# jgkellymit/GENIE-SMEM

Measured on AMD Instinct MI355X. Metric: query-bases/sec SMEM discovery, 100kb ref x 150bp reads; bit-exact SMEM set, higher is better.
Workload: dtype u8/int32 (2-bit packed bases, int32 SA rows; f64 only in the RMI predict)

## Files before the change

genie-smem_amd/csrc/kernels.hip:

```cpp
#include <hip/hip_runtime.h>

#include <algorithm>
#include <cstdio>
#include <cstdlib>
#include <mutex>
#include <string>
#include <unordered_map>

#include "genie_internal.h"

namespace genie {

namespace {

constexpr int kWave = 64;

__device__ __forceinline__ int rfl(int v) { return __builtin_amdgcn_readfirstlane(v); }
__device__ __forceinline__ void set_wave_priority(int i)
{
    switch (i & 3) {
    case 0: __builtin_amdgcn_s_setprio(0); break;
    case 1: __builtin_amdgcn_s_setprio(1); break;
    case 2: __builtin_amdgcn_s_setprio(2); break;
    default: __builtin_amdgcn_s_setprio(3); break;
    }
}

__device__ __forceinline__ void scalar_touch_lines(const void *p, uint32_t bytes)
{
    uint32_t d, off;
    asm volatile("s_mov_b32 %[off], 0\n"
                 "1:\n\t"
                 "s_load_dword %[d], %[p], %[off]\n\t"
                 "s_add_u32 %[off], %[off], 64\n\t"
                 "s_cmp_lt_u32 %[off], %[n]\n\t"
                 "s_cbranch_scc1 1b\n\t"
                 "s_waitcnt lgkmcnt(0)"
                 : [d] "=&s"(d), [off] "=&s"(off)
                 : [p] "s"(reinterpret_cast<uint64_t>(p) & ~3ull), [n] "s"(bytes)
                 : "scc", "memory");
}

__device__ __forceinline__ void wave_lds_fence()
{
    __builtin_amdgcn_fence(__ATOMIC_ACQ_REL, "wavefront");
    __builtin_amdgcn_wave_barrier();
}

__device__ __forceinline__ uint64_t funnel(uint64_t w0, uint64_t w1, int sh )
{
// ... 1 lines not shown
}

__device__ __forceinline__ uint64_t qwin(const uint64_t *qp, int pos)
{
    int i = pos >> 5;
    return funnel(qp[i], qp[i + 1], (pos & 31) * 2);
}

__device__ __forceinline__ uint64_t rwin(const RefRec *ref, int pos)
{
    const ulonglong2 v = *reinterpret_cast<const ulonglong2 *>(ref + (pos >> 5));
    return funnel(v.x, v.y, (pos & 31) * 2);
}

struct QWords {
    const uint64_t *p;
    __device__ __forceinline__ uint64_t win(int pos) const { return qwin(p, pos); }
};
struct QRecs {
    const RefRec *p;
    __device__ __forceinline__ uint64_t win(int pos) const { return rwin(p, pos); }
};
struct QPlain {
    const uint64_t *p;
    __device__ __forceinline__ uint64_t win(int pos) const
    {
        typedef uint64_t u64x2 __attribute__((ext_vector_type(2)));
        typedef u64x2 u64x2_a8 __attribute__((aligned(8)));
        const u64x2 v = *reinterpret_cast<const u64x2_a8 *>(p + (pos >> 5));
        return funnel(v.x, v.y, (pos & 31) * 2);
    }
};

template <class D>
__device__ __forceinline__ uint32_t dir_lb(const DevIndex &ix, const D dir, uint32_t code, int m)
{
    const uint32_t x = code << (2 * (ix.P - m));
    uint32_t v = dir[x];
#pragma unroll
    for (int l = 0; l < GENIE_MAX_DIR_BITS; l++)
        if (l >= m && l < ix.P && ix.padtail[l] == x) v--;
    return v;
}

template <class D>
__device__ __forceinline__ uint32_t dir_ub(const DevIndex &ix, const D dir, uint32_t code, int m)
{
    const uint32_t x = (code + 1) << (2 * (ix.P - m));
    uint32_t v = dir[x];
#pragma unroll
    for (int l = 1; l < GENIE_MAX_DIR_BITS; l++)
        if (l < ix.P && ix.padtail[l] == x) v--;
    return v;
}

struct Cmp {
    int l;
    bool less;
};

template <class Q>
__device__ __forceinline__ Cmp cmp_suffix(const DevIndex &ix, const Q qp, int a, int m, int s, int skip)
{
    const int avail = ix.n - s;
    const int lim = m < avail ? m : avail;
    int l = skip;
    bool less = false;
    bool diff = false;
    while (l < lim) {
        const uint64_t xq = qp.win(a + l), xr = rwin(ix.ref, s + l);
        const uint64_t x = xq ^ xr;
        if (x) {
            l += __clzll((long long)x) >> 1;
            less = xr < xq;
            diff = true;
            break;
        }
        l += 32;
    }
    if (!diff || l >= lim) {
        l = lim;
        less = lim < m;
    }
    return {l, less};
}

template <class Q>
__device__ __forceinline__ Cmp cmp_rec(const DevIndex &ix, const Q qp, int a, int m, const SaRec rec, uint64_t xq)
{
    const int avail = ix.n - rec.s;
    const int lim = m < avail ? m : avail;
    int l = ix.P;
    bool less;
    const uint64_t x = xq ^ rec.key;
    if (x) {
        l += __clzll((long long)x) >> 1;
        less = rec.key < xq;
        if (l >= lim) { l = lim; less = lim < m; }
    } else if (l + 32 >= lim) {
        l = lim;
        less = lim < m;
    } else {
        return cmp_suffix(ix, qp, a, m, rec.s, l + 32);
    }
    return {l, less};
}

__device__ __forceinline__ int pick_probe(int lo, int hi, uint32_t xq32, uint32_t vlo, uint32_t vhi, int step)
{
    const int n = hi - lo;
    if ((step & 1) || n <= 2 || vhi <= vlo) return (lo + hi) >> 1;
    if (xq32 <= vlo) return lo;
    if (xq32 >= vhi) return hi - 1;
    const float f = (float)(xq32 - vlo) / (float)(vhi - vlo);
    int mid = lo + (int)(f * (float)n);
    mid = mid < lo ? lo : (mid > hi - 1 ? hi - 1 : mid);
    return mid;
}

typedef uint32_t nt_u4 __attribute__((ext_vector_type(4)));
typedef nt_u4 nt_u4_unaligned __attribute__((aligned(1)));
__device__ __forceinline__ void store_nt(void *dst, uint4 v)
{
    __builtin_nontemporal_store(nt_u4{v.x, v.y, v.z, v.w}, reinterpret_cast<nt_u4 *>(dst));
}

__device__ __forceinline__ SaRec load_rec(const SaRec *sa, int row)
{
    int4 v = *reinterpret_cast<const int4 *>(sa + row);
    asm volatile("" : "+v"(v.x), "+v"(v.y), "+v"(v.z), "+v"(v.w));
    SaRec r;
    r.s = v.x;
    r.pad = 0;
    r.key = ((uint64_t)(uint32_t)v.w << 32) | (uint32_t)v.z;
    return r;
}

__device__ __forceinline__ bool lut_probe(const DevIndex &ix, uint32_t code, int &lo, int &hi)
{
    uint32_t p = (uint32_t)(((uint64_t)(code * 0x9E3779B1u) * (uint64_t)ix.lut_slots) >> 32);
    for (uint32_t tries = 0; tries < ix.lut_slots; tries++) {
        const int4 v = *reinterpret_cast<const int4 *>(ix.lut + p);
        if (v.y < 0) return false;
        if ((uint32_t)v.x == code) { lo = v.y; hi = v.z; return true; }
        p = p + 1 == ix.lut_slots ? 0 : p + 1;
    }
    return false;
}

__device__ __forceinline__ double rmi_predict(const DevIndex &ix, const RmiModel *leaf, int leaf_cnt, uint32_t code,
                                              int *leaf_idx = nullptr)
{
    const double x = (double)code;
    double p = 0.0;
    int idx = 0;
    for (int l = 0; l < ix.nlev; l++) {
        if (leaf_idx && l == ix.nlev - 1) *leaf_idx = idx;
        double2 m;
        if (leaf && l == ix.nlev - 1 && idx < leaf_cnt) m = *reinterpret_cast<const double2 *>(leaf + idx);
        else m = *reinterpret_cast<const double2 *>(ix.rmi + ix.rmi_off[l] + idx);
        p = __dadd_rn(__dmul_rn(m.x, x), m.y);
        const int scale = ix.rmi_scale[l];
        idx = !(p > 0.0) ? 0 : (p >= (double)scale ? scale - 1 : (int)p);
    }
    return p;
}

__device__ __forceinline__ int kmer_cmp_row(const DevIndex &ix, int r, uint32_t code)
{
    const int s = ix.sa[r].s;
    const int avail = ix.n - s;
    if (avail == 0) return -1;
    const uint64_t w = rwin(ix.ref, s);
    if (avail >= ix.K) {
        const uint32_t rc = (uint32_t)(w >> (64 - 2 * ix.K));
        return rc < code ? -1 : (rc > code ? 1 : 0);
    }
    const uint32_t rc = (uint32_t)(w >> (64 - 2 * avail));
    const uint32_t qc = code >> (2 * (ix.K - avail));
    return rc <= qc ? -1 : 1;
}

__device__ __forceinline__ bool rmi_lookup(const DevIndex &ix, const RmiModel *leaf, uint32_t code, int &lo, int &hi,
                                           double *pred_out)
{
    int leaf_idx = 0;
    const double p = rmi_predict(ix, leaf, 0, code, &leaf_idx);
    if (pred_out) *pred_out = p;
    const int rows = ix.n + 1;
    const int r0 = !(p > 0.0) ? 0 : (p >= (double)rows ? rows - 1 : (int)p);
    int L, R;
    bool fenced = false;
    if (ix.rmi_err) {
        const int e = ix.rmi_err[leaf_idx];
        L = r0 - e < 0 ? 0 : r0 - e;
        R = r0 + e + 1 > rows ? rows : r0 + e + 1;
        int l2 = L, r2 = R;
        while (l2 < r2) {
            const int mid = (l2 + r2) >> 1;
            if (kmer_cmp_row(ix, mid, code) < 0) l2 = mid + 1; else r2 = mid;
        }
        if (l2 < rows && kmer_cmp_row(ix, l2, code) == 0 && (l2 > L || L == 0 || kmer_cmp_row(ix, l2 - 1, code) < 0)) {
            L = R = l2;
            fenced = true;
        }
    }
    if (!fenced) {
    if (kmer_cmp_row(ix, r0, code) < 0) {
        L = r0 + 1;
        R = rows;
        for (int step = 1;; step <<= 1) {
            const int pr = r0 + step;
            if (pr >= rows) break;
            if (kmer_cmp_row(ix, pr, code) < 0) L = pr + 1;
            else { R = pr; break; }
        }
    } else {
        R = r0;
        L = 0;
        for (int step = 1;; step <<= 1) {
            const int pr = r0 - step;
            if (pr < 0) break;
            if (kmer_cmp_row(ix, pr, code) < 0) { L = pr + 1; break; }
            R = pr;
        }
    }
    }
    while (L < R) {
        const int mid = (L + R) >> 1;
        if (kmer_cmp_row(ix, mid, code) < 0) L = mid + 1; else R = mid;
    }
    const int first = L;
    if (first >= rows || kmer_cmp_row(ix, first, code) != 0) { lo = first; hi = first - 1; return false; }
    int a = first, b = rows;
    for (int step = 1;; step <<= 1) {
        const int pr = first + step;
        if (pr >= rows) break;
        if (kmer_cmp_row(ix, pr, code) == 0) a = pr;
        else { b = pr; break; }
    }
    while (b - a > 1) {
        const int mid = (a + b) >> 1;
        if (kmer_cmp_row(ix, mid, code) == 0) a = mid; else b = mid;
    }
    lo = first;
    hi = a;
    return true;
}

template <class Q>
__device__ __forceinline__ int2 sa_interval(const DevIndex &ix, const uint32_t *dir, const Q qp, int a, int m)
{
    if (m == 0) return make_int2(0, ix.n);
    const int P = ix.P;
    const uint64_t w = qp.win(a);
    if (m <= P) {
        const uint32_t code = (uint32_t)(w >> (64 - 2 * m));
        const int lb = (int)dir_lb(ix, dir, code, m), ub = (int)dir_ub(ix, dir, code, m);
        return lb < ub ? make_int2(lb, ub - 1) : make_int2(-1, -1);
    }
    const uint64_t xq = qp.win(a + P);
    int lo, hi, h;
    int known = -1;
    if (ix.P2 && m >= ix.P2) {
        int4 hd = *reinterpret_cast<const int4 *>(ix.dir2 + (uint32_t)(w >> (64 - 2 * ix.P2)));
        asm volatile("" : "+v"(hd.x), "+v"(hd.y), "+v"(hd.z), "+v"(hd.w));
        const uint32_t cnt = (uint32_t)hd.y & ~kHeadShort;
        if (cnt == 0) return make_int2(-1, -1);
        lo = hd.x;
        hi = h = hd.x + (int)cnt;
        const uint64_t key = ((uint64_t)(uint32_t)hd.w << 32) | (uint32_t)hd.z;
        const uint64_t x = xq ^ key;
        if (!((uint32_t)hd.y & kHeadShort) && (x != 0 || m <= P + 32)) {
            const int l = x ? P + (__clzll((long long)x) >> 1) : m;
            if (l >= m) { h = lo; known = lo; }
            else if (key < xq) lo = lo + 1;
            else h = lo;
        }
    } else {
        const uint32_t b = (uint32_t)(w >> (64 - 2 * P));
        lo = (int)dir[b];
        hi = h = (int)dir_ub(ix, dir, b, P);
    }
    uint32_t vlo = 0, vhi = 0xFFFFFFFFu;
// ... 930 lines not shown
```

genie-smem_amd/csrc/match_table_body.inc:

```
    static_assert(!(PK && RC), "both strands of 2-bit packed reads are not built");
    typedef uint32_t __attribute__((aligned(1))) u32_unaligned;
    extern __shared__ __align__(16) uint8_t smem[];
    const int lane = threadIdx.x & (kWave - 1);
    const int wave = rfl((int)(threadIdx.x >> 6));
    const int waves_per_block = blockDim.x >> 6;
    const int dbg = (flags >> 8) & 63;
    const int sched = flags >> 16;
    const bool look_up_all = (flags & 1) != 0;
    const int FS = fwd_stride;
    const int K = ix.K;
    const int P2 = ix.P2;
    const int DW = mt_short_row_dwords(max_len, qp_recs);
    const int DWp = mt_pack_dwords(max_len);
    const int QL = mt_quads(max_len);
    const int nquads = grp * QL;
    const __amdgpu_buffer_rsrc_t mtab =
        __builtin_amdgcn_make_buffer_rsrc(const_cast<MatchRec *>(ix.mtab), 0, (int)mtab_bytes, 0x00020000);
    const __amdgpu_buffer_rsrc_t ov =
        __builtin_amdgcn_make_buffer_rsrc(const_cast<MatchOv16 *>(ix.ov), 0, ix.ov_entries * (int)sizeof(MatchOv16), 0x00020000);

    uint8_t *wb = smem + wave * mt_wave_bytes(grp, max_len, qp_recs, FS);
    uint32_t *Dp = reinterpret_cast<uint32_t *>(wb);
    int *Ls = reinterpret_cast<int *>(wb + mt_r16(grp * DW * 4));
    uint8_t *fwL = reinterpret_cast<uint8_t *>(Ls) + 64;
    uint16_t *sl = reinterpret_cast<uint16_t *>(fwL + mt_r16(grp * FS));
    uint16_t *qa = reinterpret_cast<uint16_t *>(reinterpret_cast<uint8_t *>(sl) + mt_r16(mt_slow_cap(grp, max_len) * 2));
    uint16_t *qb = qa + grp * mt_quads(max_len);
    for (int i = lane; i < grp * DW; i += kWave) Dp[i] = 0;
    const uint8_t *reads_end = reads + (RC ? N >> 1 : N) * (long long)stride;

    const int pu = (int)(((uint32_t)lane * (uint32_t)(65536 / DWp + 1)) >> 16);
    const int pj = lane - pu * DWp;

    uint32_t *next_group = reinterpret_cast<uint32_t *>(smem + waves_per_block * mt_wave_bytes(grp, max_len, qp_recs, FS));
    const long long groups = (N + grp - 1) / grp;
    const long long share = (groups + gridDim.x - 1) / gridDim.x;
    const long long g_begin = (long long)blockIdx.x * share;
    const long long g_end = g_begin + share < groups ? g_begin + share : groups;
    const bool handed_out = !(sched & 1), rotate = !(sched & 2);
    if (threadIdx.x == 0) *next_group = (uint32_t)waves_per_block;
    uint2 *qtab = reinterpret_cast<uint2 *>(next_group + 4);
    for (int t = threadIdx.x; t < (nquads + 191) / 192 * 192; t += blockDim.x) {
        const int tq = t < nquads ? t : 0;
        const int u = tq / QL, a = 4 * (tq - u * QL);
        const uint32_t o = 2u * (uint32_t)a + 1u;
        qtab[t] = make_uint2((uint32_t)u << 28 | (uint32_t)(u * FS + a) << 16 | (uint32_t)a,
                             ((uint32_t)(u * DW) + (o >> 5)) << 8 | (32u - (o & 31u)));
    }
    __syncthreads();
    long long gi = handed_out ? g_begin + wave : (long long)blockIdx.x * waves_per_block + wave;
    const long long g_stop = handed_out ? g_end : groups;
    const int round_of_block = (int)(blockIdx.x / (uint32_t)cus);
    const bool touch_ahead = !(sched & 8);
    for (int it = 0; gi < g_stop; it++) {
        const long long r = gi * grp;
        if (rotate) set_wave_priority(it + round_of_block);
        long long gi_next;
        if (handed_out) {
            uint32_t nx = 0;
            if (lane == 0) nx = atomicAdd(next_group, 1u);
            gi_next = g_begin + (long long)(uint32_t)rfl((int)nx);
        } else {
            gi_next = gi + (long long)gridDim.x * waves_per_block;
        }
        if (touch_ahead && stride > 0 && gi_next < g_stop) {
            const long long rn = gi_next * grp;
            const long long rows = N - rn < (long long)grp ? N - rn : (long long)grp;
            if (RC) scalar_touch_lines(reads + (rn >> 1) * (long long)stride, (uint32_t)((((rn + rows - 1) >> 1) - (rn >> 1) + 1) * stride));
            else scalar_touch_lines(reads + rn * (long long)stride, (uint32_t)(rows * stride));
        }
        bool any_read = false;
        for (int u0 = 0; u0 < grp; u0 += kWave / DWp) {
            const int u = u0 + pu;
            const bool mine = pu < kWave / DWp && u < grp;
            int L = 0, st = GENIE_READ_OK;
            uint32_t d = 0;
            bool bad = false;
            if (mine && r + u < N) {
                const long long row = RC ? (r + u) >> 1 : r + u;
                const bool rev = RC && ((r + u) & 1);
                L = lens ? lens[row] : fixed_len;
                if (RC && lens && pj == 0) vlens[r + u] = L;
                if (L < 0 || L > max_len) { st = GENIE_READ_BAD_BASE; L = 0; }
                const int left = L - 16 * pj;
                if (PK) {
                    if (left > 0) {
                        d = __builtin_bswap32(*reinterpret_cast<const uint32_t *>(reads + (r + u) * (long long)stride + 4 * pj));
                        if (left < 16) d &= ~0u << (32 - 2 * left);
                    }
                }
                const uint8_t *src = reads + row * (long long)stride + 16 * pj;
                uint32_t v[4] = {0, 0, 0, 0};
                if (PK) {
                } else if (rev) {
                    const long long o = row * (long long)stride + L - 16 - 16 * pj;
                    if (left >= 16 || (left > 0 && o >= 0)) {
                        const nt_u4 q = *reinterpret_cast<const nt_u4_unaligned *>(reads + o);
                        v[0] = __builtin_bswap32(q.w); v[1] = __builtin_bswap32(q.z); v[2] = __builtin_bswap32(q.y); v[3] = __builtin_bswap32(q.x);
                        if (left < 16) {
#pragma unroll
                            for (int k = 0; k < 4; k++) {
                                const int nb = left - 4 * k;
                                v[k] = nb >= 4 ? v[k] : (nb <= 0 ? 0u : v[k] & ((1u << (8 * nb)) - 1u));
                            }
                        }
                    } else if (left > 0) {
                        const uint8_t *f = reads + row * (long long)stride;
                        for (int b = 0; b < left; b++) v[b >> 2] |= (uint32_t)f[left - 1 - b] << (8 * (b & 3));
                    }
                } else if (left >= 16 || (left > 0 && src + 16 <= reads_end)) {
                    const nt_u4 q = *reinterpret_cast<const nt_u4_unaligned *>(src);
                    v[0] = q.x; v[1] = q.y; v[2] = q.z; v[3] = q.w;
                    if (left < 16) {
#pragma unroll
                        for (int k = 0; k < 4; k++) {
                            const int nb = left - 4 * k;
                            v[k] = nb >= 4 ? v[k] : (nb <= 0 ? 0u : v[k] & ((1u << (8 * nb)) - 1u));
                        }
                    }
                } else if (left > 0) {
#pragma unroll
                    for (int k = 0; k < 4; k++) {
                        if (left >= 4 * k + 4) v[k] = *reinterpret_cast<const u32_unaligned *>(src + 4 * k);
                        else for (int b = 0; b < left - 4 * k; b++) v[k] |= (uint32_t)src[4 * k + b] << (8 * b);
                    }
                }
                if (!PK) {
                    bad = ((v[0] | v[1] | v[2] | v[3]) & 0xFCFCFCFCu) != 0;
                    d = (mt_pack4(v[0]) << 24) | (mt_pack4(v[1]) << 16) | (mt_pack4(v[2]) << 8) | mt_pack4(v[3]);
                    if (rev && left > 0) d ^= left >= 16 ? ~0u : ~0u << (32 - 2 * left);
                }
            }
            const uint32_t prev = (uint32_t)__builtin_amdgcn_update_dpp(0, (int)d, 0x138 , 0xf, 0xf, true);
            const unsigned long long badm = __ballot(bad);
            bool ok = false;
            if (mine) {
                Dp[u * DW + pj] = __builtin_amdgcn_alignbit(prev, d, 1);
                if (pj == 0) {
                    const unsigned long long mine_bits = ((1ull << DWp) - 1ull) << (pu * DWp);
                    if (st == GENIE_READ_OK && (badm & mine_bits)) st = GENIE_READ_BAD_BASE;
                    if (st == GENIE_READ_OK && mode != GENIE_MODE_BWA && L < K) st = GENIE_READ_TOO_SHORT;
                    if (r + u < N) status[r + u] = st;
                    ok = st == GENIE_READ_OK && L > 0;
                    Ls[u] = ok ? L : 0;
                }
            }
            any_read |= __any(ok);
        }
        wave_lds_fence();
        if (any_read) {
            for (int t0 = 0; t0 < ((dbg & 8) ? 0 : grp * qp_recs); t0 += kWave) {
                const int t = t0 + lane;
                const int u = t / qp_recs, i = t - u * qp_recs;
                if (t < grp * qp_recs && Ls[u] > 0) {
                    const uint32_t *q = Dp + u * DW + 4 * i;
                    const uint32_t q0 = q[0], q1 = q[1], q2 = q[2], q3 = q[3], q4 = q[4];
                    uint4 rec;
                    rec.y = __builtin_amdgcn_alignbit(q0, q1, 31);
                    rec.x = __builtin_amdgcn_alignbit(q1, q2, 31);
                    rec.w = __builtin_amdgcn_alignbit(q2, q3, 31);
                    rec.z = __builtin_amdgcn_alignbit(q3, q4, 31);
                    store_nt(qp_out + (r + u) * (long long)qp_stride + i, rec);
                }
            }
            int nslow = 0;
            int positions = grp * max_len;
            asm volatile("" : "+s"(positions));
            const int flush_at = positions > kMtSlowCap ? kMtSlowCap - kWave : 1 << 30;
            const int n1 = (dbg & 4) ? 0 : nquads;
            int c0 = 0;
            do {
#pragma nounroll
            for (; c0 < n1 && nslow + (kMtNsp - 1) * kWave <= flush_at; c0 += kMtNsp * kWave) {
                uint32_t ent[kMtNsp];
                MtProbe pr[kMtNsp];
#pragma unroll
                for (int s = 0; s < kMtNsp; s++) {
                    const int t0 = c0 + 64 * s + lane;
                    const uint2 q = qtab[t0];
                    int m = Ls[q.x >> 28] - (int)(q.x & 255u);
                    m = t0 < nquads && m > 0 ? m : 0;
                    ent[s] = q.x | ((uint32_t)m << 8);
                    const uint32_t *dq = Dp + (q.y >> 8);
                    const uint32_t sh = q.y & 255u;
                    const uint32_t d0 = dq[0], d1 = dq[1], d2 = dq[2];
                    pr[s] = mt_issue<C16>(mtab, __builtin_amdgcn_alignbit(d0, d1, sh), __builtin_amdgcn_alignbit(d1, d2, sh), P2);
                }
                mt_v4i rb[kMtNsp];
#pragma unroll
                for (int s = 0; s < kMtNsp; s++) rb[s] = mt_second<C16>(mtab, pr[s]);
#pragma unroll
                for (int s = 0; s < kMtNsp; s++) {
                    bool slow;
                    const int best0 = mt_eval<C16>(pr[s], rb[s], P2, slow);
                    const int a = (int)(ent[s] & 255u), m = (int)((ent[s] >> 8) & 255u);
                    const int best = best0 < m ? best0 : m;
                    if (m) fwL[(ent[s] >> 16) & 0xFFFu] = (uint8_t)(a + best);
                    slow = slow && m > best0;
                    const unsigned long long sb = __ballot(slow);
                    if (slow) sl[nslow + __popcll(sb & ((1ull << lane) - 1ull))] = (uint16_t)(((ent[s] >> 28) << 8) | (uint32_t)a);
                    nslow += __popcll(sb);
                }
            }
            wave_lds_fence();
#pragma nounroll
            for (int s0 = 0; s0 < ((dbg & 1) ? 0 : nslow); s0 += kWave) mt_slow<false, C16>(ix, mtab, ov, mode, lane, s0, nslow, sl, Dp, DW, Ls, fwL, FS);
            wave_lds_fence();
            nslow = 0;
            } while (__builtin_expect(c0 < n1, 0));
            int nqa = 0, nqb = 0;
            const unsigned long long below = (1ull << lane) - 1ull;
#pragma nounroll
            for (int t0 = lane; t0 < ((dbg & 6) ? 0 : nquads) + lane; t0 += kWave) {
                const uint2 q = qtab[t0 < nquads ? t0 : 0];
                const int u = (int)(q.x >> 28), a = (int)(q.x & 255u);
                const int L = Ls[u];
                const int m = t0 < nquads && L > a ? L - a : 0;
                const uint32_t fo = (q.x >> 16) & 0xFFFu;
                const uint32_t v0 = fwL[fo];
                const bool has_right = m > 4;
                const uint32_t v4 = has_right ? fwL[fo + 4] : 0u;
                const bool need = m > 1 && (look_up_all || ((int)v0 != L && !(has_right && v4 == v0)));
                if (m && !need) *reinterpret_cast<uint32_t *>(fwL + fo) = v0 * 0x01010101u;
                const unsigned long long nb = __ballot(need);
                if (need) qa[nqa + __popcll(nb & below)] = (uint16_t)((uint32_t)u << 8 | (uint32_t)a);
                nqa += __popcll(nb);
            }
            wave_lds_fence();
            int cm = 0, cn = 0;
            do {
#pragma nounroll
            for (; cm < nqa && nslow <= flush_at; cm += kWave) {
                const bool valid = cm + lane < nqa;
                const uint32_t it = qa[valid ? cm + lane : 0];
                const int u = (int)(it >> 8), a = (int)(it & 255u);
                const int L = Ls[u], m = L - a;
                const int km = m > 2 ? 2 : 1;
                const uint32_t fo = __umul24((uint32_t)u, (uint32_t)FS) + (uint32_t)a;
                const uint32_t o = 2u * (uint32_t)(a + km) + 1u;
                const uint32_t *dq = Dp + __umul24((uint32_t)u, (uint32_t)DW) + (o >> 5);
                const uint32_t sh = 32u - (o & 31u);
                const uint32_t d0 = dq[0], d1 = dq[1], d2 = dq[2];
                const MtProbe pm = mt_issue<C16>(mtab, __builtin_amdgcn_alignbit(d0, d1, sh), __builtin_amdgcn_alignbit(d1, d2, sh), P2);
                const uint32_t v0 = fwL[fo];
                const bool has_right = m > 4;
                const uint32_t v4 = has_right ? fwL[fo + 4] : 0u;
                const mt_v4i rm = mt_second<C16>(mtab, pm);
                bool sm;
                const int bm = mt_eval<C16>(pm, rm, P2, sm);
                const int em = bm < m - km ? bm : m - km;
                sm = valid && sm && m - km > bm;
                const uint32_t vm = (uint32_t)(a + km + em);
                bool need1 = false, need3 = false;
                if (valid) {
                    if (km == 1) {
                        *reinterpret_cast<uint32_t *>(fwL + fo) = v0 | vm << 8;
                    } else {
                        need1 = look_up_all || sm || vm != v0;
                        need3 = m > 3 && (look_up_all || sm || !((has_right && vm == v4) || (int)vm == L));
                        *reinterpret_cast<uint32_t *>(fwL + fo) = v0 | v0 << 8 | vm << 16 | (m > 3 ? vm : 0u) << 24;
                    }
                }
                const unsigned long long sbm = __ballot(sm), b1 = __ballot(need1), b3 = __ballot(need3);
                if (sm) sl[nslow + __popcll(sbm & below)] = (uint16_t)(it + (uint32_t)km);
                nslow += __popcll(sbm);
                if (need1) qb[nqb + __popcll(b1 & below)] = (uint16_t)(it + 1u);
                nqb += __popcll(b1);
                if (need3) qb[nqb + __popcll(b3 & below)] = (uint16_t)(it + 3u);
                nqb += __popcll(b3);
            }
            wave_lds_fence();
#pragma nounroll
            for (; cm >= nqa && cn < nqb && nslow <= flush_at; cn += kWave) {
                const bool valid = cn + lane < nqb;
                const uint32_t it = qb[valid ? cn + lane : 0];
                const int u = (int)(it >> 8), a = (int)(it & 255u);
                const int m = Ls[u] - a;
                const uint32_t o = 2u * (uint32_t)a + 1u;
                const uint32_t *dq = Dp + __umul24((uint32_t)u, (uint32_t)DW) + (o >> 5);
                const uint32_t sh = 32u - (o & 31u);
                const uint32_t d0 = dq[0], d1 = dq[1], d2 = dq[2];
                const MtProbe pn = mt_issue<C16>(mtab, __builtin_amdgcn_alignbit(d0, d1, sh), __builtin_amdgcn_alignbit(d1, d2, sh), P2);
                const mt_v4i rn = mt_second<C16>(mtab, pn);
                bool slow;
                const int b0 = mt_eval<C16>(pn, rn, P2, slow);
                const int e = b0 < m ? b0 : m;
                if (valid) fwL[__umul24((uint32_t)u, (uint32_t)FS) + (uint32_t)a] = (uint8_t)(a + e);
                slow = valid && slow && m > b0;
                const unsigned long long sb = __ballot(slow);
                if (slow) sl[nslow + __popcll(sb & below)] = (uint16_t)it;
                nslow += __popcll(sb);
            }
            wave_lds_fence();
#pragma nounroll
            for (int s0 = 0; s0 < ((dbg & 1) ? 0 : nslow); s0 += kWave) mt_slow<false, C16>(ix, mtab, ov, mode, lane, s0, nslow, sl, Dp, DW, Ls, fwL, FS);
            wave_lds_fence();
            nslow = 0;
            } while (__builtin_expect(cm < nqa || cn < nqb, 0));
            const int nrows = N - r < (long long)grp ? (int)(N - r) : grp;
            uint4 *dst = reinterpret_cast<uint4 *>(fwd_out + r * (long long)FS);
            const uint4 *src = reinterpret_cast<const uint4 *>(fwL);
            for (int i = lane; i < ((dbg & 32) ? 0 : nrows * (FS >> 4)); i += kWave) store_nt(dst + i, src[i]);
        }
        wave_lds_fence();
        gi = gi_next;
    }
```

genie-smem_amd/csrc/match_table_kernel.inc:

```

constexpr int kMtNsp = 3;
constexpr int kMtMaxG = 16;
constexpr int kMtTarget = 768;
constexpr int kMtTarget2 = 1536;
constexpr int kMtSlowCap = 512;


__host__ __device__ inline int mt_row_dwords(int max_len, int qp_recs)
{
    const int a = ((2 * (max_len + 8) + 1) >> 5) + 3, b = 2 * qp_recs + 3;
    return a > b ? a : b;
}
__host__ __device__ inline int mt_pack_dwords(int max_len) { return (max_len + 15) / 16 + 1; }
__host__ __device__ inline int mt_quads(int max_len) { return (max_len + 3) / 4; }
__host__ __device__ inline int mt_r16(int x) { return (x + 15) & ~15; }
__host__ __device__ inline int mt_quad_table_bytes(int grp, int max_len) { return (grp * mt_quads(max_len) + 191) / 192 * 192 * 8; }
__host__ __device__ inline int mt_short_row_dwords(int max_len, int chunks) { return mt_row_dwords(max_len, 2 * chunks - 1); }
__host__ __device__ inline int mt_slow_cap(int grp, int max_len) { return grp * max_len <= kMtSlowCap ? grp * max_len : kMtSlowCap; }
__host__ __device__ inline int mt_wave_bytes(int grp, int max_len, int qp_recs, int fwd_stride)
{
    return mt_r16(grp * mt_short_row_dwords(max_len, qp_recs) * 4) + 64 + mt_r16(grp * fwd_stride) + mt_r16(mt_slow_cap(grp, max_len) * 2) +
           mt_r16(grp * mt_quads(max_len) * 6);
}

// ... 92 lines not shown
    if (km == 1) {
        q.v1 = vm;
        q.s1 = sm;
        return q;
    }
    q.v2 = vm;
    q.s2 = sm;
    const bool need1 = look_up_all || sm || vm != v0;
    const bool need3 = m > 3 && (look_up_all || sm || !((has_right && vm == v4) || (int)vm == L));
    q.v1 = v0;
    q.v3 = m > 3 ? vm : 0u;
    if (need1 || need3) {
        const uint32_t s13 = need1 ? sh - 2 : sh - 6;
        const MtProbe pa = mt_issue<C16>(mtab, __builtin_amdgcn_alignbit(d0, d1, s13), __builtin_amdgcn_alignbit(d1, d2, s13), P2);
        MtProbe pb = pa;
        const bool both = need1 && need3;
        if (both) pb = mt_issue<C16>(mtab, __builtin_amdgcn_alignbit(d0, d1, sh - 6), __builtin_amdgcn_alignbit(d1, d2, sh - 6), P2);
        const mt_v4i ra = mt_second<C16>(mtab, pa);
        mt_v4i rb = ra;
        if (both) rb = mt_second<C16>(mtab, pb);
        bool sa, sb;
        const int ba = mt_eval<C16>(pa, ra, P2, sa), bb = mt_eval<C16>(pb, rb, P2, sb);
        const int ka = need1 ? 1 : 3;
        const int ea = ba < m - ka ? ba : m - ka, eb = bb < m - 3 ? bb : m - 3;
        sa = sa && m - ka > ba;
        sb = sb && m - 3 > bb;
        if (need1) { q.v1 = (uint32_t)(a + 1 + ea); q.s1 = sa; }
        else { q.v3 = (uint32_t)(a + 3 + ea); q.s3 = sa; }
        if (both) { q.v3 = (uint32_t)(a + 3 + eb); q.s3 = sb; }
    }
    return q;
}

template <bool LONG, bool C16, class QB = QBits, class FW = uint16_t>
__device__ __forceinline__ void mt_slow(const DevIndex &ix, const __amdgpu_buffer_rsrc_t mtab, const __amdgpu_buffer_rsrc_t ov, int mode, int lane, int c0,
                                        int count, const uint16_t *list, const uint32_t *Dp, int DW, const int *Ls,
                                        uint8_t *fwL, int FS, int L0 = 0, int wbase = 0, FW *fwW = nullptr)
{
    const int K = ix.K, P = ix.P, P2 = ix.P2;
    const int idx = c0 + lane;
    const bool on = idx < count;
    int u = 0, a = 0, m = 0, best = 0, chain = 0, cvoff = 0, nrows = 0;
    uint32_t mask = 0, lb = 0, c = 0, xmin = ~0u, xkq = 0;
    bool general = false;
    uint64_t w = 0, xq = 0;
    QB Q{reinterpret_cast<decltype(QB::p)>(Dp)};
    if (on) {
        const uint32_t e = (uint32_t)list[idx];
        if constexpr (LONG) {
            a = wbase + (int)e;
            m = L0 - a;
        } else {
            u = (int)(e >> 8);
            a = (int)(e & 255u);
            m = Ls[u] - a;
            Q.p = Dp + u * DW;
        }
        w = Q.win(a);
        xq = Q.win(a + P);
        c = (uint32_t)(w >> (64 - 2 * P2));
        const uint32_t xk = (uint32_t)((w << (2 * P2)) >> 32);
        if (C16) {
            const mt_v4i e = __builtin_amdgcn_raw_buffer_load_b128(mtab, (int)(c << 4), 0, 0);
            const uint32_t w0 = (uint32_t)e.x, cnt4 = (w0 >> 24) & 15u, xk16 = xk >> 16;
            lb = w0 & 0xFFFFFFu;
            best = P2;
            const uint32_t total = cnt4 == kM16More ? 7u + (w0 >> 28) : cnt4;
            const bool wide = ((w0 >> 28) & kM16Wide) && cnt4 >= 1u && cnt4 <= 3u;
// ... 66 lines not shown
    if (chain) {
        const int lcp = __clz((int)xmin) >> 1;
        const int l = P2 + lcp < m ? P2 + lcp : m;
        best = l > best ? l : best;
        if (lcp < 16 || m <= P2 + 16) mask = 0;
        else mask &= nrows >= 32 ? ~0u : (1u << nrows) - 1u;
    }
    while (__any(mask != 0)) {
        if (mask) {
            const int i = __ffs((int)mask) - 1;
            mask &= mask - 1;
            const Cmp r = cmp_rec(ix, Q, a, m, load_rec(ix.sa, (int)lb + i), xq);
            best = r.l > best ? r.l : best;
        }
    }
    if (__any(general)) {
        int lo = 0, hi = 0, hint = -1;
        if (general) {
            int4 hd = *reinterpret_cast<const int4 *>(ix.dir2 + c);
            asm volatile("" : "+v"(hd.x), "+v"(hd.y), "+v"(hd.z), "+v"(hd.w));
            const uint32_t cnt = (uint32_t)hd.y & ~kHeadShort;
            lo = hd.x;
            hi = hd.x + (int)cnt;
            const uint64_t key = ((uint64_t)(uint32_t)hd.w << 32) | (uint32_t)hd.z;
            const uint64_t x = xq ^ key;
            if (!((uint32_t)hd.y & kHeadShort) && (x != 0 || m <= P + 32)) {
                int l = x ? P + (__clzll((long long)x) >> 1) : m;
                bool less = key < xq;
                if (l >= m) { l = m; less = false; }
                best = l > best ? l : best;
                if (less) lo = hd.x + 1; else hi = hd.x;
            }
            if (mode == GENIE_MODE_RMI && m >= K && K >= P2) {
                const double p = rmi_predict(ix, nullptr, 0, (uint32_t)(w >> (64 - 2 * K)));
                hint = !(p > 0.0) ? 0 : (p >= (double)ix.n ? ix.n : (int)p);
            }
        }
        while (__any(lo < hi)) {
            if (lo < hi) {
                int mid = (lo + hi) >> 1;
                if (hint >= lo && hint < hi) mid = hint;
                hint = -1;
                const Cmp r = cmp_rec(ix, Q, a, m, load_rec(ix.sa, mid), xq);
                best = r.l > best ? r.l : best;
                if (r.less) lo = mid + 1; else hi = mid;
            }
        }
    }
    if (on) {
        if (LONG) fwW[a - wbase] = (FW)(a + best);
        else fwL[u * FS + a] = (uint8_t)(a + best);
    }
}

template <int WPS, bool C16, bool PK>
__global__ void __launch_bounds__(512, WPS) match_table_kernel(DevIndex ix, int mode, const uint8_t *__restrict__ reads,
                                                             const int32_t *__restrict__ lens, long long N, int stride,
                                                             int fixed_len, uint8_t *__restrict__ fwd_out, int fwd_stride,
                                                             RefRec *__restrict__ qp_out, int qp_recs, int qp_stride,
                                                             int32_t *__restrict__ status, int grp, int max_len,
                                                             long long mtab_bytes, int flags, int cus)
{
    constexpr bool RC = false;
    int32_t *const vlens = nullptr;
#include "match_table_body.inc"
}
template <int WPS, bool C16>
// ... 43 lines not shown
```

genie-smem_amd/csrc/short_read_kernel.inc:

```

template <bool WIDE>
struct ReadTraits {
    typedef uint8_t fwd_t;
    static constexpr int kj_bits = 16, kj_shift = 8;
};
template <>
struct ReadTraits<true> {
    typedef uint16_t fwd_t;
    static constexpr int kj_bits = 32, kj_shift = 16;
};


typedef unsigned short kb_us2 __attribute__((ext_vector_type(2)));
__device__ __forceinline__ uint32_t kb_pk_max(uint32_t a, uint32_t b)
{
    return __builtin_bit_cast(uint32_t, __builtin_elementwise_max(__builtin_bit_cast(kb_us2, a), __builtin_bit_cast(kb_us2, b)));
}

constexpr int kPairHeadWords = 4;

__device__ __forceinline__ int block_exclusive_scan(int v, int &total)
{
    __shared__ int wave_total[16];
    const int lane = threadIdx.x & (kWave - 1), wave = threadIdx.x >> 6;
// ... 294 lines not shown

struct RowEscapes {
    unsigned long long *count;
    long long *list;
    long long cap;
};
template <int COUT>
__device__ __forceinline__ void emit_row(void *out, long long idx, int k, int j, int lo, int hi, const RowEscapes &esc)
{
    if (COUT == 0) {
        store_nt(reinterpret_cast<int4 *>(out) + idx, make_uint4((uint32_t)k, (uint32_t)j, (uint32_t)lo, (uint32_t)hi));
        return;
    }
    constexpr uint32_t kTop = COUT == 1 ? 0xFFFFu : 0xFFu;
    uint32_t span = (uint32_t)(hi - lo);
    if (span >= kTop) {
        const unsigned long long slot = atomicAdd(esc.count, 1ull);
        if ((long long)slot < esc.cap) {
            esc.list[2 * slot] = idx;
            esc.list[2 * slot + 1] = hi;
        }
        span = kTop;
    }
    if (COUT == 1) {
        reinterpret_cast<uint2 *>(out)[idx] = make_uint2((uint32_t)k | (uint32_t)j << 8 | span << 16, (uint32_t)lo);
    } else {
        uint16_t *o = reinterpret_cast<uint16_t *>(out) + 3 * idx;
        o[0] = (uint16_t)((uint32_t)k | (uint32_t)j << 8);
        o[1] = (uint16_t)lo;
        o[2] = (uint16_t)(((uint32_t)lo >> 16) | span << 8);
    }
}

template <bool C16>
__device__ __forceinline__ bool interval_from_entry(const int4 ra, const int4 rb, uint64_t w, int len, int P2,
                                                    const __amdgpu_buffer_rsrc_t ov, bool act, int2 &iv)
{
    const uint32_t meta = (uint32_t)ra.x;
    bool fast = false;
    iv = make_int2(-1, -1);
    if (C16) {
        const uint32_t cnt4 = (meta >> 24) & 15u, nib = meta >> 28, lb = meta & 0xFFFFFFu;
        if (act && cnt4 == 0) {
            if (len == (int)nib) { fast = true; iv = make_int2((int)lb, ra.y); }
        } else if (act && (nib & kM16Wide) && cnt4 <= 3u && len >= P2) {
            const uint32_t xk = (uint32_t)((w << (2 * P2)) >> 32);
            const int cl = len - P2 < 16 ? len - P2 : 16;
            const uint32_t km = cl == 0 ? 0u : ~0u << (32 - 2 * cl);
            const uint32_t bits = (((((uint32_t)ra.y ^ xk) & km) == 0 ? 1u : 0u) | ((((uint32_t)ra.z ^ xk) & km) == 0 ? 2u : 0u) |
                                   ((((uint32_t)ra.w ^ xk) & km) == 0 ? 4u : 0u)) & ((1u << cnt4) - 1u);
            fast = len <= P2 + 16 || __popc(bits) == 1;
            if (bits) {
                const int first = (int)lb + __ffs((int)bits) - 1;
                iv = make_int2(first, first + __popc(bits) - 1);
            }
        } else if (act && (cnt4 == kM16More || !(nib & kM16General)) && len >= P2) {
            const uint32_t total = cnt4 == kM16More ? 7u + nib : cnt4;
            const uint32_t xk16 = (uint32_t)((w << (2 * P2)) >> 48);
            const int cl = len - P2 < 8 ? len - P2 : 8;
            const uint32_t km16 = cl == 0 ? 0u : (0xFFFFu << (16 - 2 * cl)) & 0xFFFFu;
            const uint32_t k16[6] = {(uint32_t)ra.y & 0xFFFFu, (uint32_t)ra.y >> 16, (uint32_t)ra.z & 0xFFFFu,
                                     (uint32_t)ra.z >> 16, (uint32_t)ra.w & 0xFFFFu, (uint32_t)ra.w >> 16};
            const uint32_t ninl = cnt4 == kM16More ? (uint32_t)kM16Keys - 1u : cnt4;
            uint32_t bits = 0, xm = 0xFFFFu;
#pragma unroll
            for (int i = 0; i < kM16Keys; i++) bits |= (((k16[i] ^ xk16) & km16) == 0 && (uint32_t)i < ninl) ? 1u << i : 0u;
            if (cnt4 == kM16More) mt_ov_scan(ov, k16[5], (int)total - (kM16Keys - 1), xk16, km16, xm, bits);
            fast = len <= P2 + 8 || __popc(bits) == 1;
            if (bits) {
                const int first = (int)lb + __ffs((int)bits) - 1;
                iv = make_int2(first, first + __popc(bits) - 1);
            }
        }
    } else if (act && !(meta & kMatchSlow)) {
        const uint32_t rows = meta >> 24;
        if (rows == 0) {
            if (len == (int)(meta & 0xFFu)) { fast = true; iv = make_int2(ra.y, ra.z); }
        } else if (len >= P2) {
            const uint32_t xk = (uint32_t)((w << (2 * P2)) >> 32);
            const int cl = len - P2 < 16 ? len - P2 : 16;
            const uint32_t km = cl == 0 ? 0u : ~0u << (32 - 2 * cl);
            uint32_t bits = ((((uint32_t)ra.z ^ xk) & km) == 0 ? 1u : 0u) | ((((uint32_t)ra.w ^ xk) & km) == 0 ? 2u : 0u) |
                            ((((uint32_t)rb.x ^ xk) & km) == 0 ? 4u : 0u) | ((((uint32_t)rb.y ^ xk) & km) == 0 ? 8u : 0u) |
                            ((((uint32_t)rb.z ^ xk) & km) == 0 ? 16u : 0u) | ((((uint32_t)rb.w ^ xk) & km) == 0 ? 32u : 0u);
            bits &= (1u << rows) - 1u;
            fast = len <= P2 + 16 || __popc(bits) == 1;
            if (bits) {
                const int first = (int)ra.y + __ffs((int)bits) - 1;
                iv = make_int2(first, first + __popc(bits) - 1);
            }
        }
    }
    return fast;
}

__device__ __forceinline__ __amdgpu_buffer_rsrc_t mt_ov_rsrc(const DevIndex &ix)
{
    return __builtin_amdgcn_make_buffer_rsrc(const_cast<MatchOv16 *>(ix.ov), 0, ix.ov_entries * (int)sizeof(MatchOv16), 0x00020000);
}

template <bool C16>
__device__ __forceinline__ void mt_load_entry(const DevIndex &ix, uint32_t code, bool act, int4 &ra, int4 &rb)
{
    const int4 *en = C16 ? reinterpret_cast<const int4 *>(reinterpret_cast<const MatchRec16 *>(ix.mtab) + code)
                         : reinterpret_cast<const int4 *>(ix.mtab + code);
    ra = make_int4(0, 0, 0, 0);
    rb = make_int4(0, 0, 0, 0);
    if (act) { ra = en[0]; if (!C16) rb = en[1]; }
}

template <bool C16>
__device__ __forceinline__ bool interval_from_window(const DevIndex &ix, uint64_t w, int len, bool act, int2 &iv)
{
    int4 ra, rb;
    mt_load_entry<C16>(ix, (uint32_t)(w >> (64 - 2 * ix.P2)), act, ra, rb);
    return interval_from_entry<C16>(ra, rb, w, len, ix.P2, mt_ov_rsrc(ix), act, iv);
}

template <int COUT, class QIn>
struct WaveList {
    const DevIndex &ix;
    const RefRec *qp_in;
    int qp_stride;
    void *out;
    RowEscapes esc;
    int4 *list;
    int nlist;

    __device__ __forceinline__ void search(int o, int n) const
    {
        const int lane = threadIdx.x & (kWave - 1);
        if (lane < n) {
            const int4 en = list[o + lane];
            const int k = en.w & 0xFFFF, j = (int)((uint32_t)en.w >> 16);
            const QIn qp{reinterpret_cast<decltype(QIn::p)>(qp_in + (long long)en.z * qp_stride)};
            const int2 iv = sa_interval(ix, ix.dir, qp, k, j - k);
            emit_row<COUT>(out, ((long long)en.y << 32) | (uint32_t)en.x, k, j, iv.x, iv.y, esc);
        }
    }
    __device__ __forceinline__ void append(bool general, long long row, int read, int k, int j)
    {
        const int lane = threadIdx.x & (kWave - 1);
        const unsigned long long gb = __ballot(general);
        if (gb) {
            if (general)
                list[nlist + __popcll(gb & ((1ull << lane) - 1ull))] = make_int4((int)(uint32_t)row, (int)(row >> 32), read, k | (j << 16));
            nlist += __popcll(gb);
            wave_lds_fence();
            if (nlist >= 64) {
                nlist -= 64;
                search(nlist, 64);
                wave_lds_fence();
            }
        }
    }
    __device__ __forceinline__ void drain() const
    {
        if (nlist) search(0, nlist);
    }
};

template <bool C16, int COUT, class QIn>
__device__ __forceinline__ void resolve_row(bool act, uint64_t w, int k, int j, long long row, int read, WaveList<COUT, QIn> &wl)
{
    int2 iv;
    const bool fast = interval_from_window<C16>(wl.ix, w, j - k, act, iv);
    if (fast) emit_row<COUT>(wl.out, row, k, j, iv.x, iv.y, wl.esc);
    wl.append(act && !fast, row, read, k, j);
}

template <bool CSR, bool WIDE, bool C16>
__global__ void __launch_bounds__(kIvWaves * 64, 8) interval_kernel(DevIndex ix, long long N,
                                                                    const void *__restrict__ kj_in, int kj_stride,
                                                                    const uint8_t *__restrict__ head_in, int head_stride,
                                                                    const RefRec *__restrict__ qp_in, int qp_stride,
                                                                    void *__restrict__ out, int cap,
                                                                    long long *__restrict__ offsets, long long out_cap,
                                                                    const unsigned long long *__restrict__ block_base,
                                                                    const int32_t *__restrict__ before_in_block, int block_shift,
                                                                    int sched)
{
    static_assert(WIDE || !CSR, "short reads, CSR rows: interval_rows_kernel");
    __shared__ int4 lists[kIvWaves][kIvList];
    typedef typename std::conditional<WIDE, uint32_t, uint16_t>::type kj_t;
    typedef typename std::conditional<WIDE, QRecs, QPlain>::type QIn;
    constexpr int kHeadEntries = kPairHeadWords * 8 / (int)sizeof(kj_t), kShift = ReadTraits<WIDE>::kj_shift;
    const int lane = threadIdx.x & (kWave - 1);
    const int wave = rfl((int)(threadIdx.x >> 6));
    const int sub = lane & 15;
    WaveList<0, QIn> wl{ix, qp_in, qp_stride, out, RowEscapes{}, lists[wave], 0};
    const long long step = (long long)gridDim.x * kIvWaves * 4;
    const bool rotate = !(sched & 1);
    int it = (int)(blockIdx.x / (uint32_t)(sched >> 8));
    for (long long r0 = ((long long)blockIdx.x * kIvWaves + wave) * 4; r0 < N; r0 += step, it++) {
        if (rotate) set_wave_priority(it);
        const bool have = r0 + (lane >> 4) < N;
        const long long r = have ? r0 + (lane >> 4) : 0;
        const kj_t *head = reinterpret_cast<const kj_t *>(head_in + r * (long long)head_stride);
        int c = have ? (int)head[0] : 0;
// ... 113 lines not shown
```

Before: 217.4 billion.

## Rematerialize index fields from kernarg pointer to cut SGPR pressure

Rarely used DevIndex fields (overflow buffer resource, dir, ref) are now read through the kernarg segment pointer in slow paths, instead of being held live in SGPRs for the whole kernel. Flag bits are re-read through opaque SGPR copies rather than being decoded into booleans up front. Per-row addressing is hoisted and the row bound is computed once per group. The aim is lower scalar register pressure and fewer spills in the match-table and interval kernels, at the cost of extra scalar loads on the slow paths.

```diff
diff --git a/genie-smem_amd/csrc/kernels.hip b/genie-smem_amd/csrc/kernels.hip
--- a/genie-smem_amd/csrc/kernels.hip
+++ b/genie-smem_amd/csrc/kernels.hip
@@ -16,6 +16,18 @@
 constexpr int kWave = 64;
 
 __device__ __forceinline__ int rfl(int v) { return __builtin_amdgcn_readfirstlane(v); }
+__device__ __forceinline__ int sgpr_opaque(int v)
+{
+    asm volatile("" : "+s"(v));
+    return v;
+}
+typedef const __attribute__((address_space(4))) DevIndex KargIndex;
+__device__ __forceinline__ KargIndex *karg_index()
+{
+    KargIndex *p = (KargIndex *)__builtin_amdgcn_kernarg_segment_ptr();
+    asm volatile("" : "+s"(p));
+    return p;
+}
 __device__ __forceinline__ void set_wave_priority(int i)
 {
     switch (i & 3) {
@@ -83,8 +95,8 @@
     }
 };
 
-template <class D>
-__device__ __forceinline__ uint32_t dir_lb(const DevIndex &ix, const D dir, uint32_t code, int m)
+template <class D, class IX>
+__device__ __forceinline__ uint32_t dir_lb(const IX &ix, const D dir, uint32_t code, int m)
 {
     const uint32_t x = code << (2 * (ix.P - m));
     uint32_t v = dir[x];
@@ -94,8 +106,8 @@
     return v;
 }
 
-template <class D>
-__device__ __forceinline__ uint32_t dir_ub(const DevIndex &ix, const D dir, uint32_t code, int m)
+template <class D, class IX>
+__device__ __forceinline__ uint32_t dir_ub(const IX &ix, const D dir, uint32_t code, int m)
 {
     const uint32_t x = (code + 1) << (2 * (ix.P - m));
     uint32_t v = dir[x];
@@ -110,8 +122,8 @@
     bool less;
 };
 
-template <class Q>
-__device__ __forceinline__ Cmp cmp_suffix(const DevIndex &ix, const Q qp, int a, int m, int s, int skip)
+template <class Q, class IX>
+__device__ __forceinline__ Cmp cmp_suffix(const IX &ix, const Q qp, int a, int m, int s, int skip)
 {
     const int avail = ix.n - s;
     const int lim = m < avail ? m : avail;
@@ -136,8 +148,8 @@
     return {l, less};
 }
 
-template <class Q>
-__device__ __forceinline__ Cmp cmp_rec(const DevIndex &ix, const Q qp, int a, int m, const SaRec rec, uint64_t xq)
+template <class Q, class IX>
+__device__ __forceinline__ Cmp cmp_rec(const IX &ix, const Q qp, int a, int m, const SaRec rec, uint64_t xq)
 {
     const int avail = ix.n - rec.s;
     const int lim = m < avail ? m : avail;
@@ -199,17 +211,15 @@
     return false;
 }
 
-__device__ __forceinline__ double rmi_predict(const DevIndex &ix, const RmiModel *leaf, int leaf_cnt, uint32_t code,
-                                              int *leaf_idx = nullptr)
+template <class IX>
+__device__ __forceinline__ double rmi_predict(const IX &ix, uint32_t code, int *leaf_idx = nullptr)
 {
     const double x = (double)code;
     double p = 0.0;
     int idx = 0;
     for (int l = 0; l < ix.nlev; l++) {
         if (leaf_idx && l == ix.nlev - 1) *leaf_idx = idx;
-        double2 m;
-        if (leaf && l == ix.nlev - 1 && idx < leaf_cnt) m = *reinterpret_cast<const double2 *>(leaf + idx);
-        else m = *reinterpret_cast<const double2 *>(ix.rmi + ix.rmi_off[l] + idx);
+        const double2 m = *reinterpret_cast<const double2 *>(ix.rmi + ix.rmi_off[l] + idx);
         p = __dadd_rn(__dmul_rn(m.x, x), m.y);
         const int scale = ix.rmi_scale[l];
         idx = !(p > 0.0) ? 0 : (p >= (double)scale ? scale - 1 : (int)p);
@@ -236,7 +246,7 @@
                                            double *pred_out)
 {
     int leaf_idx = 0;
-    const double p = rmi_predict(ix, leaf, 0, code, &leaf_idx);
+    const double p = rmi_predict(ix, code, &leaf_idx);
     if (pred_out) *pred_out = p;
     const int rows = ix.n + 1;
     const int r0 = !(p > 0.0) ? 0 : (p >= (double)rows ? rows - 1 : (int)p);
@@ -299,8 +309,8 @@
     return true;
 }
 
-template <class Q>
-__device__ __forceinline__ int2 sa_interval(const DevIndex &ix, const uint32_t *dir, const Q qp, int a, int m)
+template <class Q, class IX>
+__device__ __forceinline__ int2 sa_interval(const IX &ix, const uint32_t *dir, const Q qp, int a, int m)
 {
     if (m == 0) return make_int2(0, ix.n);
     const int P = ix.P;
diff --git a/genie-smem_amd/csrc/match_table_body.inc b/genie-smem_amd/csrc/match_table_body.inc
--- a/genie-smem_amd/csrc/match_table_body.inc
+++ b/genie-smem_amd/csrc/match_table_body.inc
@@ -4,9 +4,9 @@
     const int lane = threadIdx.x & (kWave - 1);
     const int wave = rfl((int)(threadIdx.x >> 6));
     const int waves_per_block = blockDim.x >> 6;
-    const int dbg = (flags >> 8) & 63;
-    const int sched = flags >> 16;
-    const bool look_up_all = (flags & 1) != 0;
+#define MT_OPT(bits) ((sgpr_opaque(flags) & (bits)) != 0)
+#define MT_DBG(bits) MT_OPT((bits) << 8)
+#define MT_SCHED(bits) MT_OPT((bits) << 16)
     const int FS = fwd_stride;
     const int K = ix.K;
     const int P2 = ix.P2;
@@ -16,8 +16,6 @@
     const int nquads = grp * QL;
     const __amdgpu_buffer_rsrc_t mtab =
         __builtin_amdgcn_make_buffer_rsrc(const_cast<MatchRec *>(ix.mtab), 0, (int)mtab_bytes, 0x00020000);
-    const __amdgpu_buffer_rsrc_t ov =
-        __builtin_amdgcn_make_buffer_rsrc(const_cast<MatchOv16 *>(ix.ov), 0, ix.ov_entries * (int)sizeof(MatchOv16), 0x00020000);
 
     uint8_t *wb = smem + wave * mt_wave_bytes(grp, max_len, qp_recs, FS);
     uint32_t *Dp = reinterpret_cast<uint32_t *>(wb);
@@ -37,7 +35,7 @@
     const long long share = (groups + gridDim.x - 1) / gridDim.x;
     const long long g_begin = (long long)blockIdx.x * share;
     const long long g_end = g_begin + share < groups ? g_begin + share : groups;
-    const bool handed_out = !(sched & 1), rotate = !(sched & 2);
+    const bool handed_out = !(flags & (1 << 16));
     if (threadIdx.x == 0) *next_group = (uint32_t)waves_per_block;
     uint2 *qtab = reinterpret_cast<uint2 *>(next_group + 4);
     for (int t = threadIdx.x; t < (nquads + 191) / 192 * 192; t += blockDim.x) {
@@ -50,20 +48,19 @@
     __syncthreads();
     long long gi = handed_out ? g_begin + wave : (long long)blockIdx.x * waves_per_block + wave;
     const long long g_stop = handed_out ? g_end : groups;
-    const int round_of_block = (int)(blockIdx.x / (uint32_t)cus);
-    const bool touch_ahead = !(sched & 8);
-    for (int it = 0; gi < g_stop; it++) {
+    for (int it = (int)(blockIdx.x / (uint32_t)cus); gi < g_stop; it++) {
         const long long r = gi * grp;
-        if (rotate) set_wave_priority(it + round_of_block);
+        const int nrows = N - r < (long long)grp ? (int)(N - r) : grp;
+        if (!MT_SCHED(2)) set_wave_priority(it);
         long long gi_next;
-        if (handed_out) {
+        if (!MT_SCHED(1)) {
             uint32_t nx = 0;
             if (lane == 0) nx = atomicAdd(next_group, 1u);
             gi_next = g_begin + (long long)(uint32_t)rfl((int)nx);
         } else {
             gi_next = gi + (long long)gridDim.x * waves_per_block;
         }
-        if (touch_ahead && stride > 0 && gi_next < g_stop) {
+        if (!MT_SCHED(8) && sgpr_opaque(stride) > 0 && gi_next < g_stop) {
             const long long rn = gi_next * grp;
             const long long rows = N - rn < (long long)grp ? N - rn : (long long)grp;
             if (RC) scalar_touch_lines(reads + (rn >> 1) * (long long)stride, (uint32_t)((((rn + rows - 1) >> 1) - (rn >> 1) + 1) * stride));
@@ -71,16 +68,18 @@
         }
         bool any_read = false;
         for (int u0 = 0; u0 < grp; u0 += kWave / DWp) {
+            const int32_t *lens_u = lens;
+            asm volatile("" : "+s"(lens_u));
             const int u = u0 + pu;
             const bool mine = pu < kWave / DWp && u < grp;
             int L = 0, st = GENIE_READ_OK;
             uint32_t d = 0;
             bool bad = false;
-            if (mine && r + u < N) {
+            if (mine && u < nrows) {
                 const long long row = RC ? (r + u) >> 1 : r + u;
                 const bool rev = RC && ((r + u) & 1);
-                L = lens ? lens[row] : fixed_len;
-                if (RC && lens && pj == 0) vlens[r + u] = L;
+                L = lens_u ? lens_u[row] : fixed_len;
+                if (RC && lens_u && pj == 0) vlens[r + u] = L;
                 if (L < 0 || L > max_len) { st = GENIE_READ_BAD_BASE; L = 0; }
                 const int left = L - 16 * pj;
                 if (PK) {
@@ -89,7 +88,7 @@
                         if (left < 16) d &= ~0u << (32 - 2 * left);
                     }
                 }
-                const uint8_t *src = reads + row * (long long)stride + 16 * pj;
+                const uint8_t *src = (RC ? reads + row * (long long)stride : reads + r * (long long)stride + (long long)u * stride) + 16 * pj;
                 uint32_t v[4] = {0, 0, 0, 0};
                 if (PK) {
                 } else if (rev) {
@@ -139,8 +138,8 @@
                 if (pj == 0) {
                     const unsigned long long mine_bits = ((1ull << DWp) - 1ull) << (pu * DWp);
                     if (st == GENIE_READ_OK && (badm & mine_bits)) st = GENIE_READ_BAD_BASE;
-                    if (st == GENIE_READ_OK && mode != GENIE_MODE_BWA && L < K) st = GENIE_READ_TOO_SHORT;
-                    if (r + u < N) status[r + u] = st;
+                    if (st == GENIE_READ_OK && sgpr_opaque(mode) != GENIE_MODE_BWA && L < K) st = GENIE_READ_TOO_SHORT;
+                    if (u < nrows) status[r + u] = st;
                     ok = st == GENIE_READ_OK && L > 0;
                     Ls[u] = ok ? L : 0;
                 }
@@ -149,7 +148,7 @@
         }
         wave_lds_fence();
         if (any_read) {
-            for (int t0 = 0; t0 < ((dbg & 8) ? 0 : grp * qp_recs); t0 += kWave) {
+            for (int t0 = 0; t0 < (MT_DBG(8) ? 0 : grp * qp_recs); t0 += kWave) {
                 const int t = t0 + lane;
                 const int u = t / qp_recs, i = t - u * qp_recs;
                 if (t < grp * qp_recs && Ls[u] > 0) {
@@ -160,14 +159,14 @@
                     rec.x = __builtin_amdgcn_alignbit(q1, q2, 31);
                     rec.w = __builtin_amdgcn_alignbit(q2, q3, 31);
                     rec.z = __builtin_amdgcn_alignbit(q3, q4, 31);
-                    store_nt(qp_out + (r + u) * (long long)qp_stride + i, rec);
+                    store_nt(qp_out + r * (long long)qp_stride + (u * qp_stride + i), rec);
                 }
             }
             int nslow = 0;
             int positions = grp * max_len;
             asm volatile("" : "+s"(positions));
             const int flush_at = positions > kMtSlowCap ? kMtSlowCap - kWave : 1 << 30;
-            const int n1 = (dbg & 4) ? 0 : nquads;
+            const int n1 = MT_DBG(4) ? 0 : nquads;
             int c0 = 0;
             do {
 #pragma nounroll
@@ -204,14 +203,17 @@
             }
             wave_lds_fence();
 #pragma nounroll
-            for (int s0 = 0; s0 < ((dbg & 1) ? 0 : nslow); s0 += kWave) mt_slow<false, C16>(ix, mtab, ov, mode, lane, s0, nslow, sl, Dp, DW, Ls, fwL, FS);
+            for (int s0 = 0; s0 < (MT_DBG(1) ? 0 : nslow); s0 += kWave) {
+                KargIndex &kix = *karg_index();
+                mt_slow<false, C16>(kix, mtab, mt_ov_rsrc(kix), sgpr_opaque(mode), lane, s0, nslow, sl, Dp, DW, Ls, fwL, FS);
+            }
             wave_lds_fence();
             nslow = 0;
             } while (__builtin_expect(c0 < n1, 0));
             int nqa = 0, nqb = 0;
             const unsigned long long below = (1ull << lane) - 1ull;
 #pragma nounroll
-            for (int t0 = lane; t0 < ((dbg & 6) ? 0 : nquads) + lane; t0 += kWave) {
+            for (int t0 = lane; t0 < (MT_DBG(6) ? 0 : nquads) + lane; t0 += kWave) {
                 const uint2 q = qtab[t0 < nquads ? t0 : 0];
                 const int u = (int)(q.x >> 28), a = (int)(q.x & 255u);
                 const int L = Ls[u];
@@ -220,7 +222,7 @@
                 const uint32_t v0 = fwL[fo];
                 const bool has_right = m > 4;
                 const uint32_t v4 = has_right ? fwL[fo + 4] : 0u;
-                const bool need = m > 1 && (look_up_all || ((int)v0 != L && !(has_right && v4 == v0)));
+                const bool need = m > 1 && (MT_OPT(1) || ((int)v0 != L && !(has_right && v4 == v0)));
                 if (m && !need) *reinterpret_cast<uint32_t *>(fwL + fo) = v0 * 0x01010101u;
                 const unsigned long long nb = __ballot(need);
                 if (need) qa[nqa + __popcll(nb & below)] = (uint16_t)((uint32_t)u << 8 | (uint32_t)a);
@@ -256,6 +258,7 @@
                     if (km == 1) {
                         *reinterpret_cast<uint32_t *>(fwL + fo) = v0 | vm << 8;
                     } else {
+                        const bool look_up_all = MT_OPT(1);
                         need1 = look_up_all || sm || vm != v0;
                         need3 = m > 3 && (look_up_all || sm || !((has_right && vm == v4) || (int)vm == L));
                         *reinterpret_cast<uint32_t *>(fwL + fo) = v0 | v0 << 8 | vm << 16 | (m > 3 ? vm : 0u) << 24;
@@ -293,15 +296,20 @@
             }
             wave_lds_fence();
 #pragma nounroll
-            for (int s0 = 0; s0 < ((dbg & 1) ? 0 : nslow); s0 += kWave) mt_slow<false, C16>(ix, mtab, ov, mode, lane, s0, nslow, sl, Dp, DW, Ls, fwL, FS);
+            for (int s0 = 0; s0 < (MT_DBG(1) ? 0 : nslow); s0 += kWave) {
+                KargIndex &kix = *karg_index();
+                mt_slow<false, C16>(kix, mtab, mt_ov_rsrc(kix), sgpr_opaque(mode), lane, s0, nslow, sl, Dp, DW, Ls, fwL, FS);
+            }
             wave_lds_fence();
             nslow = 0;
             } while (__builtin_expect(cm < nqa || cn < nqb, 0));
-            const int nrows = N - r < (long long)grp ? (int)(N - r) : grp;
             uint4 *dst = reinterpret_cast<uint4 *>(fwd_out + r * (long long)FS);
             const uint4 *src = reinterpret_cast<const uint4 *>(fwL);
-            for (int i = lane; i < ((dbg & 32) ? 0 : nrows * (FS >> 4)); i += kWave) store_nt(dst + i, src[i]);
+            for (int i = lane; i < (MT_DBG(32) ? 0 : nrows * (FS >> 4)); i += kWave) store_nt(dst + i, src[i]);
         }
         wave_lds_fence();
         gi = gi_next;
     }
+#undef MT_OPT
+#undef MT_DBG
+#undef MT_SCHED
diff --git a/genie-smem_amd/csrc/match_table_kernel.inc b/genie-smem_amd/csrc/match_table_kernel.inc
--- a/genie-smem_amd/csrc/match_table_kernel.inc
+++ b/genie-smem_amd/csrc/match_table_kernel.inc
@@ -148,8 +148,8 @@
     return q;
 }
 
-template <bool LONG, bool C16, class QB = QBits, class FW = uint16_t>
-__device__ __forceinline__ void mt_slow(const DevIndex &ix, const __amdgpu_buffer_rsrc_t mtab, const __amdgpu_buffer_rsrc_t ov, int mode, int lane, int c0,
+template <bool LONG, bool C16, class QB = QBits, class FW = uint16_t, class IX>
+__device__ __forceinline__ void mt_slow(const IX &ix, const __amdgpu_buffer_rsrc_t mtab, const __amdgpu_buffer_rsrc_t ov, int mode, int lane, int c0,
                                         int count, const uint16_t *list, const uint32_t *Dp, int DW, const int *Ls,
                                         uint8_t *fwL, int FS, int L0 = 0, int wbase = 0, FW *fwW = nullptr)
 {
@@ -282,7 +282,7 @@
                 if (less) lo = hd.x + 1; else hi = hd.x;
             }
             if (mode == GENIE_MODE_RMI && m >= K && K >= P2) {
-                const double p = rmi_predict(ix, nullptr, 0, (uint32_t)(w >> (64 - 2 * K)));
+                const double p = rmi_predict(ix, (uint32_t)(w >> (64 - 2 * K)));
                 hint = !(p > 0.0) ? 0 : (p >= (double)ix.n ? ix.n : (int)p);
             }
         }
diff --git a/genie-smem_amd/csrc/short_read_kernel.inc b/genie-smem_amd/csrc/short_read_kernel.inc
--- a/genie-smem_amd/csrc/short_read_kernel.inc
+++ b/genie-smem_amd/csrc/short_read_kernel.inc
@@ -350,9 +350,11 @@
     }
 }
 
-template <bool C16>
+struct OvFromKarg {};
+__device__ __forceinline__ __amdgpu_buffer_rsrc_t ov_rsrc_of(const __amdgpu_buffer_rsrc_t ov) { return ov; }
+template <bool C16, class OV>
 __device__ __forceinline__ bool interval_from_entry(const int4 ra, const int4 rb, uint64_t w, int len, int P2,
-                                                    const __amdgpu_buffer_rsrc_t ov, bool act, int2 &iv)
+                                                    const OV ov, bool act, int2 &iv)
 {
     const uint32_t meta = (uint32_t)ra.x;
     bool fast = false;
@@ -383,7 +385,7 @@
             uint32_t bits = 0, xm = 0xFFFFu;
 #pragma unroll
             for (int i = 0; i < kM16Keys; i++) bits |= (((k16[i] ^ xk16) & km16) == 0 && (uint32_t)i < ninl) ? 1u << i : 0u;
-            if (cnt4 == kM16More) mt_ov_scan(ov, k16[5], (int)total - (kM16Keys - 1), xk16, km16, xm, bits);
+            if (cnt4 == kM16More) mt_ov_scan(ov_rsrc_of(ov), k16[5], (int)total - (kM16Keys - 1), xk16, km16, xm, bits);
             fast = len <= P2 + 8 || __popc(bits) == 1;
             if (bits) {
                 const int first = (int)lb + __ffs((int)bits) - 1;
@@ -412,7 +414,8 @@
     return fast;
 }
 
-__device__ __forceinline__ __amdgpu_buffer_rsrc_t mt_ov_rsrc(const DevIndex &ix)
+template <class IX>
+__device__ __forceinline__ __amdgpu_buffer_rsrc_t mt_ov_rsrc(const IX &ix)
 {
     return __builtin_amdgcn_make_buffer_rsrc(const_cast<MatchOv16 *>(ix.ov), 0, ix.ov_entries * (int)sizeof(MatchOv16), 0x00020000);
 }
@@ -427,12 +430,15 @@
     if (act) { ra = en[0]; if (!C16) rb = en[1]; }
 }
 
-template <bool C16>
+__device__ __forceinline__ __amdgpu_buffer_rsrc_t ov_rsrc_of(OvFromKarg) { return mt_ov_rsrc(*karg_index()); }
+
+template <bool C16, bool KARG = false>
 __device__ __forceinline__ bool interval_from_window(const DevIndex &ix, uint64_t w, int len, bool act, int2 &iv)
 {
     int4 ra, rb;
     mt_load_entry<C16>(ix, (uint32_t)(w >> (64 - 2 * ix.P2)), act, ra, rb);
-    return interval_from_entry<C16>(ra, rb, w, len, ix.P2, mt_ov_rsrc(ix), act, iv);
+    if constexpr (KARG) return interval_from_entry<C16>(ra, rb, w, len, ix.P2, OvFromKarg{}, act, iv);
+    else return interval_from_entry<C16>(ra, rb, w, len, ix.P2, mt_ov_rsrc(ix), act, iv);
 }
 
 template <int COUT, class QIn>
@@ -452,7 +458,8 @@
             const int4 en = list[o + lane];
             const int k = en.w & 0xFFFF, j = (int)((uint32_t)en.w >> 16);
             const QIn qp{reinterpret_cast<decltype(QIn::p)>(qp_in + (long long)en.z * qp_stride)};
-            const int2 iv = sa_interval(ix, ix.dir, qp, k, j - k);
+            KargIndex &kix = *karg_index();
+            const int2 iv = sa_interval(kix, kix.dir, qp, k, j - k);
             emit_row<COUT>(out, ((long long)en.y << 32) | (uint32_t)en.x, k, j, iv.x, iv.y, esc);
         }
     }
@@ -482,7 +489,7 @@
 __device__ __forceinline__ void resolve_row(bool act, uint64_t w, int k, int j, long long row, int read, WaveList<COUT, QIn> &wl)
 {
     int2 iv;
-    const bool fast = interval_from_window<C16>(wl.ix, w, j - k, act, iv);
+    const bool fast = interval_from_window<C16, true>(wl.ix, w, j - k, act, iv);
     if (fast) emit_row<COUT>(wl.out, row, k, j, iv.x, iv.y, wl.esc);
     wl.append(act && !fast, row, read, k, j);
 }
```

Measured after the change: 214.7 billion. 0.987x the previous value.
